# thilinarmtb/lsbench

Measured on AMD Instinct MI355X. Metric: cg_solves_per_sec, higher is better.
Workload: dtype f64

## Files before the change

lsbench_amd/csrc/hip_kernels.hip:

```cpp
#include "hip_kcommon.h"

__device__ __forceinline__ void spmv_publish(double *__restrict__ partials, double dot,
                                             double *sred, const lsb_ar_tail &tail) {
  if (!partials)
    return;
  double d[1] = {dot};
  wg_sum<1>(d, sred);
  if (tail.counter)
    ar_tail(partials, d[0], tail);
  else if (threadIdx.x == 0)
    partials[blockIdx.x] = d[0];
}

enum { SP_PREFETCH = 1, SP_NT = 2 };

template <int FLAGS, class T>
__device__ __forceinline__ T stream_load(const T *p) {
  if (FLAGS & SP_NT)
    return __builtin_nontemporal_load(p);
  return *p;
}

#define LSB_ISSUE_BLOCK(kk)                                                    \
  do {                                                                         \
// ... 602 lines not shown
        edge = x[e];
      }
      if (!have_xd && !(dot_is_x && bc == 0)) {
        if (row + 1 < n)
          xd = *(const sell_d2v *)(xdot + row);
        else if (row < n)
          xd.x = xdot[row];
        have_xd = true;
      }
      unsigned long long mk[2][2] = {{0ull, 0ull}, {0ull, 0ull}};
#pragma unroll
      for (int side = 0; side < 2; side++)
        if (side_k[side] >= 0 && side_kd[side] == 2) {
          const unsigned long long *mp = mask + 2 * ((size_t)mb + (unsigned)side_k[side]);
          mk[side][0] = mp[0], mk[side][1] = mp[1];
        }
      TMPL_UNPARK();
      if (stopped)
        return;
      double up = lane_above(c.y), dn = lane_below(c.x);
      if (lane == 0)
        up = edge;
      if (lane == 63)
        dn = edge;
      if (!have_xd)
        xd.x = c.x, xd.y = c.y, have_xd = true;
#pragma unroll
      for (int k = 0; k < NF; k++) {
        const double v = T->cst[k];
        a0 = fma(v, lo[k].x, a0), a1 = fma(v, lo[k].y, a1);
      }
      {
        double vm0 = T->cst[NF], vm1 = vm0, vp0 = T->cst[NF + 2], vp1 = vp0;
        if (side_k[0] >= 0 || side_k[1] >= 0)
          tmpl_side_values(T, NF, vb, lane, side_k, side_kd, mk, vals, f32, vm0, vm1, vp0, vp1);
        const double vc = T->cst[NF + 1];
        a0 = fma(vm0, vm0 != 0.0 ? up : 0.0, a0), a1 = fma(vm1, vm1 != 0.0 ? c.x : 0.0, a1);
        a0 = fma(vc, c.x, a0), a1 = fma(vc, c.y, a1);
        a0 = fma(vp0, vp0 != 0.0 ? c.y : 0.0, a0), a1 = fma(vp1, vp1 != 0.0 ? dn : 0.0, a1);
      }
#pragma unroll
      for (int k = 0; k < NF; k++) {
        const double v = T->cst[NF + 3 + k];
        a0 = fma(v, hi[k].x, a0), a1 = fma(v, hi[k].y, a1);
      }
    } else {
      TMPL_UNPARK();
      if (!have_xd) {
        if (row + 1 < n)
          xd = *(const sell_d2v *)(xdot + row);
        else if (row < n)
          xd.x = xdot[row];
        have_xd = true;
      }
      if (t != 255u) {
        const int cnt = T->nslots;
        if (stopped)
          return;
        for (int u0 = 0; u0 < LSB_TMPL_SLOTS; u0 += 4) {
          sell_d2u v[4];
#pragma unroll
          for (int u = 0; u < 4; u++)
            if (u0 + u < cnt)
              v[u] = *(const sell_d2u *)(x + (grow + T->base[u0 + u]));
#pragma unroll
          for (int u = 0; u < 4; u++)
            if (u0 + u < cnt) {
              const double k = T->cst[u0 + u];
              a0 = fma(k, v[u].x, a0), a1 = fma(k, v[u].y, a1);
            }
        }
      } else {
        const unsigned q0 = sptr[s] / LSB_SELL_ROWS, len = (sptr[s + 1] - sptr[s]) / LSB_SELL_ROWS;
        if (stopped)
          return;
        for (unsigned j = 0; j < len; j++) {
          const i4v r = ((const i4v *)sbase)[q0 + j];
          if (r.z < 0) {
            const double k = vconst[q0 + j];
            const sell_d2u v = *(const sell_d2u *)(x + (grow + r.x));
            a0 = fma(k, v.x, a0), a1 = fma(k, v.y, a1);
          } else {
            double v0, v1;
            if (f32) {
              const vt2<float>::type v = *((const vt2<float>::type *)((const float *)vals + (size_t)r.z * LSB_SELL_ROWS) + lane);
              v0 = (double)v.x, v1 = (double)v.y;
            } else {
              const sell_d2v v = *((const sell_d2v *)((const double *)vals + (size_t)r.z * LSB_SELL_ROWS) + lane);
              v0 = v.x, v1 = v.y;
            }
            const bool p0 = v0 != 0.0, p1 = v1 != 0.0;
            const double t0 = x[p0 ? grow + r.x : 0], t1 = x[p1 ? grow + 1 + r.x : 0];
            a0 = fma(v0, p0 ? t0 : 0.0, a0), a1 = fma(v1, p1 ? t1 : 0.0, a1);
          }
        }
      }
    }
    if (CHEB) {
      if (row + 1 < n) {
        const sell_d2v rr = *(const sell_d2v *)(epi.r + row), dd = *(const sell_d2v *)(epi.d + row);
        const double i0 = epi.dinv ? epi.dinv[row] : epi.dc, i1 = epi.dinv ? epi.dinv[row + 1] : epi.dc;
        const double v0 = fma(epi.a, dd.x, epi.b * (i0 * (rr.x - a0)));
        const double v1 = fma(epi.a, dd.y, epi.b * (i1 * (rr.y - a1)));
        const sell_d2v dn2 = {v0, v1}, zn = {x[grow] + v0, x[grow + 1] + v1};
        *(sell_d2v *)(epi.d + row) = dn2;
        *(sell_d2v *)(epi.zout + row) = zn;
      } else if (row < n) {
        const double v0 = fma(epi.a, epi.d[row], epi.b * ((epi.dinv ? epi.dinv[row] : epi.dc) * (epi.r[row] - a0)));
        epi.d[row] = v0;
        epi.zout[row] = x[grow] + v0;
      }
    } else if (DEFER && s * LSB_SELL_ROWS + LSB_SELL_ROWS <= n) {
      const sell_d2v o = {a0, a1};
      if (DEFER_DEPTH == 1 || pslot == 0)
        ypark[tid] = o, parked[0] = s * LSB_SELL_ROWS;
      else
        ypark[(DEFER_DEPTH - 1) * WG + tid] = o, parked[DEFER_DEPTH - 1] = s * LSB_SELL_ROWS;
      if (xdot) {
        dot = fma(a0, xd.x, dot);
        dot = fma(a1, xd.y, dot);
      }
    } else if (row + 1 < n) {
      const sell_d2v o = {a0, a1};
      *(sell_d2v *)(y + row) = o;
      if (xdot) {
        dot = fma(a0, xd.x, dot);
        dot = fma(a1, xd.y, dot);
      }
    } else if (row < n) {
      y[row] = a0;
      if (xdot)
        dot = fma(a0, xd.x, dot);
    }
  }
#pragma unroll
  for (int k = 0; k < DEFER_DEPTH; k++)
    TMPL_UNPARK_SLOT(k);
#undef TMPL_UNPARK
#undef TMPL_UNPARK_SLOT
  if (stopped)
    return;
  spmv_publish(partials, dot, sred, tail);
}

template <int NF> struct col_ops {
  sell_d2u lo[NF > 1 ? NF - 1 : 1], hi[NF > 1 ? NF - 1 : 1];
  double edge;
  sell_d2v xd;
};
template <int NF> struct col_tmpl {
  int bc, bl[NF > 1 ? NF - 1 : 1], bh[NF > 1 ? NF - 1 : 1];
  double k0, kl[NF > 1 ? NF - 1 : 1], kc, kh[NF > 1 ? NF - 1 : 1], kL;
};
template <int NF, int DOT>
__device__ __forceinline__ void col_issue(col_ops<NF> &o, sell_d2u &cnext, const col_tmpl<NF> &T, const double *__restrict__ x,
                                          const double *__restrict__ xdot, long long gu, unsigned lrow, long long D,
                                          unsigned xlen, unsigned lane, bool with_next) {
  if (with_next)
    cnext = *(const sell_d2u *)(x + (gu + T.bc + D) + 2 * lane);
#pragma unroll
  for (int k = 0; k < NF - 1; k++) {
    o.lo[k] = *(const sell_d2u *)(x + (gu + T.bl[k]) + 2 * lane);
    o.hi[k] = *(const sell_d2u *)(x + (gu + T.bh[k]) + 2 * lane);
  }
  long long el = gu + T.bc - 1, er = gu + T.bc + (long long)LSB_SELL_ROWS;
  el = el < 0 ? 0 : el, er = er >= (long long)xlen ? (long long)xlen - 1 : er;
  o.edge = x[lane < 32u ? el : er];
  if (DOT == 2)
    o.xd = *(const sell_d2v *)(xdot + lrow + 2 * lane);
}
template <int NF, int DOT>
__device__ __forceinline__ void col_compute(const col_ops<NF> &o, const sell_d2u &cm, const sell_d2u &c, const sell_d2u &cp,
                                            const col_tmpl<NF> &T, double vm0, double vm1, double vp0, double vp1,
                                            unsigned lane, double &a0, double &a1, double &dot) {
  double up = lane_above(c.y), dn = lane_below(c.x);
  if (lane == 0)
    up = o.edge;
  if (lane == 63)
    dn = o.edge;
  a0 = fma(T.k0, cm.x, 0.0), a1 = fma(T.k0, cm.y, 0.0);
#pragma unroll
  for (int k = 0; k < NF - 1; k++)
    a0 = fma(T.kl[k], o.lo[k].x, a0), a1 = fma(T.kl[k], o.lo[k].y, a1);
  a0 = fma(vm0, vm0 != 0.0 ? up : 0.0, a0), a1 = fma(vm1, vm1 != 0.0 ? c.x : 0.0, a1);
  a0 = fma(T.kc, c.x, a0), a1 = fma(T.kc, c.y, a1);
  a0 = fma(vp0, vp0 != 0.0 ? c.y : 0.0, a0), a1 = fma(vp1, vp1 != 0.0 ? dn : 0.0, a1);
#pragma unroll
  for (int k = 0; k < NF - 1; k++)
    a0 = fma(T.kh[k], o.hi[k].x, a0), a1 = fma(T.kh[k], o.hi[k].y, a1);
  a0 = fma(T.kL, cp.x, a0), a1 = fma(T.kL, cp.y, a1);
  if (DOT == 1)
    dot = fma(a0, c.x, dot), dot = fma(a1, c.y, dot);
  else if (DOT == 2)
    dot = fma(a0, o.xd.x, dot), dot = fma(a1, o.xd.y, dot);
}

#define LSB_COL_HEAD 16
__device__ __forceinline__ bool col_walks_down(const unsigned *__restrict__ plan, unsigned dofs, unsigned it) {
  return dofs && ((plan[dofs + (it >> 5)] >> (it & 31u)) & 1u);
}
template <int NF, int DOT>
__global__ __launch_bounds__(WG, DOT == 2 ? 5 : 6) void k_spmv_tmpl_col(
    const unsigned *__restrict__ plan, unsigned period, unsigned n, unsigned row_begin, unsigned xlen,
    const unsigned *__restrict__ sptr, const unsigned long long *__restrict__ mask,
    const lsb_sell_tmpl *__restrict__ td, const int *__restrict__ sbase, const void *__restrict__ vals, int f32,
    const double *__restrict__ vconst, const double *__restrict__ x, double *__restrict__ y,
    const double *__restrict__ xdot, double *__restrict__ partials, const lsb_pcg_state *__restrict__ st,
    const lsb_ar_tail tail) {
  static_assert(NF >= 1 && NF <= 2, "one or two far slots per side");
  __shared__ double sred[4];
  const unsigned tid = threadIdx.x, lane = tid & 63u, wave = tid >> 6;
  const unsigned gx = gridDim.x / NXCD, xcd = blockIdx.x % NXCD, slot = blockIdx.x / NXCD;
  const unsigned i0 = plan[xcd], i1 = plan[xcd + 1];
  const u4v *__restrict__ items = (const u4v *)(plan + LSB_COL_HEAD);
  const unsigned dofs = plan[LSB_TMPL_COL_DOWN];
  const int stopped = st ? st->status : 0;
  const unsigned P = period * LSB_SELL_ROWS;
  double dot = 0.0;
  for (unsigned g = slot; i0 + 4 * g < i1; g += gx) {
    const unsigned it = __builtin_amdgcn_readfirstlane(i0 + 4 * g + wave);
    if (it >= i1)
      continue;
    const u4v rec = items[it];
    const unsigned s = __builtin_amdgcn_readfirstlane(rec.x), Kw = __builtin_amdgcn_readfirstlane(rec.y);
    const unsigned K = Kw & ~LSB_TMPL_COL_LOCKSTEP;
    const bool lockstep = (Kw & LSB_TMPL_COL_LOCKSTEP) != 0;
    if (K >= 2) {
      const unsigned t = __builtin_amdgcn_readfirstlane(rec.z), mb = __builtin_amdgcn_readfirstlane(rec.w);
      const lsb_sell_tmpl *T = td + t;
      col_tmpl<NF> C;
      C.bc = T->base[NF + 1];
      C.k0 = T->cst[0], C.kc = T->cst[NF + 1], C.kL = T->cst[2 * NF + 2];
#pragma unroll
      for (int k = 0; k < NF - 1; k++) {
        C.bl[k] = T->base[1 + k], C.bh[k] = T->base[NF + 3 + k];
        C.kl[k] = T->cst[1 + k], C.kh[k] = T->cst[NF + 3 + k];
      }
      const int side_k[2] = {T->kidx[NF], T->kidx[NF + 2]}, side_kd[2] = {T->kind[NF], T->kind[NF + 2]};
      unsigned long long mk[2][2] = {{0ull, 0ull}, {0ull, 0ull}};
#pragma unroll
      for (int side = 0; side < 2; side++)
        if (side_k[side] >= 0 && side_kd[side] == 2) {
          const unsigned long long *mp = mask + 2 * ((size_t)mb + (unsigned)side_k[side]);
          mk[side][0] = mp[0], mk[side][1] = mp[1];
        }
      const bool down = col_walks_down(plan, dofs, it);
      const unsigned s0 = down ? s + (K - 1) * period : s;
      const long long D = down ? -(long long)P : (long long)P;
      const unsigned Du = (unsigned)D;
      long long gu = (long long)s0 * LSB_SELL_ROWS + row_begin;
      unsigned lrow = s0 * LSB_SELL_ROWS;
      col_ops<NF> cur, nxt;
      sell_d2u cb = *(const sell_d2u *)(x + (gu + C.bc - D) + 2 * lane);
      sell_d2u c0 = *(const sell_d2u *)(x + (gu + C.bc) + 2 * lane);
      sell_d2u ca, cn;
      col_issue<NF, DOT>(cur, ca, C, x, xdot, gu, lrow, D, xlen, lane, true);
      double vm0 = T->cst[NF], vm1 = vm0, vp0 = T->cst[NF + 2], vp1 = vp0;
      if (side_k[0] >= 0 || side_k[1] >= 0)
        tmpl_side_values(T, NF, 0u, lane, side_k, side_kd, mk, vals, f32, vm0, vm1, vp0, vp1);
      if (stopped)
        return;
      col_issue<NF, DOT>(nxt, cn, C, x, xdot, gu + D, lrow + Du, D, xlen, lane, true);
      double a0, a1;
      col_compute<NF, DOT>(cur, down ? ca : cb, c0, down ? cb : ca, C, vm0, vm1, vp0, vp1, lane, a0, a1, dot);
      cb = c0, c0 = ca, ca = cn, cur = nxt;
      for (unsigned k = 1; k + 1 < K; k++) {
        gu += D, lrow += Du;
        if (lockstep)
          __builtin_amdgcn_s_barrier();
        col_issue<NF, DOT>(nxt, cn, C, x, xdot, gu + D, lrow + Du, D, xlen, lane, true);
        {
          const sell_d2v o = {a0, a1};
          *(sell_d2v *)(y + (lrow - Du) + 2 * lane) = o;
        }
        col_compute<NF, DOT>(cur, down ? ca : cb, c0, down ? cb : ca, C, vm0, vm1, vp0, vp1, lane, a0, a1, dot);
        cb = c0, c0 = ca, ca = cn, cur = nxt;
      }
      gu += D, lrow += Du;
      {
        const sell_d2v o = {a0, a1};
        *(sell_d2v *)(y + (lrow - Du) + 2 * lane) = o;
      }
      col_compute<NF, DOT>(cur, down ? ca : cb, c0, down ? cb : ca, C, vm0, vm1, vp0, vp1, lane, a0, a1, dot);
      {
        const sell_d2v o = {a0, a1};
        *(sell_d2v *)(y + lrow + 2 * lane) = o;
      }
      if (stopped)
        return;
    } else {
      const unsigned row = s * LSB_SELL_ROWS + 2 * lane;
      const int grow = (int)(row + row_begin);
      const unsigned q0 = sptr[s] / LSB_SELL_ROWS, len = (sptr[s + 1] - sptr[s]) / LSB_SELL_ROWS;
      sell_d2v xd = {0.0, 0.0};
      if (DOT) {
        if (row + 1 < n)
          xd = *(const sell_d2v *)(xdot + row);
        else if (row < n)
          xd.x = xdot[row];
      }
      if (stopped)
        return;
      double a0 = 0.0, a1 = 0.0;
      for (unsigned j = 0; j < len; j++) {
        const i4v r = ((const i4v *)sbase)[q0 + j];
        if (r.z < 0) {
          const double k = vconst[q0 + j];
          const sell_d2u v = *(const sell_d2u *)(x + (grow + r.x));
          a0 = fma(k, v.x, a0), a1 = fma(k, v.y, a1);
        } else {
          double v0, v1;
          if (f32) {
            const vt2<float>::type v = *((const vt2<float>::type *)((const float *)vals + (size_t)r.z * LSB_SELL_ROWS) + lane);
            v0 = (double)v.x, v1 = (double)v.y;
          } else {
            const sell_d2v v = *((const sell_d2v *)((const double *)vals + (size_t)r.z * LSB_SELL_ROWS) + lane);
            v0 = v.x, v1 = v.y;
          }
          const bool p0 = v0 != 0.0, p1 = v1 != 0.0;
          const double t0 = x[p0 ? grow + r.x : 0], t1 = x[p1 ? grow + 1 + r.x : 0];
          a0 = fma(v0, p0 ? t0 : 0.0, a0), a1 = fma(v1, p1 ? t1 : 0.0, a1);
        }
      }
      if (row + 1 < n) {
        const sell_d2v o = {a0, a1};
        *(sell_d2v *)(y + row) = o;
        if (DOT)
          dot = fma(a0, xd.x, dot), dot = fma(a1, xd.y, dot);
      } else if (row < n) {
        y[row] = a0;
        if (DOT)
          dot = fma(a0, xd.x, dot);
      }
    }
  }
  if (stopped)
    return;
  spmv_publish(partials, dot, sred, tail);
}

template <int NF> struct colp_c {
  sell_d2u rn, pn;
  sell_d2v xn, sn;
  double re, pe;
};
template <int NF> struct colp_m {
  sell_d2u rlo[NF > 1 ? NF - 1 : 1], plo[NF > 1 ? NF - 1 : 1], rhi[NF > 1 ? NF - 1 : 1], phi[NF > 1 ? NF - 1 : 1];
};
struct colp_out {
  sell_d2v q, x, p;
};
template <int NF, bool WITH_X, int NT>
__device__ __forceinline__ void colp_issue_c(colp_c<NF> &o, const col_tmpl<NF> &T, const double *__restrict__ r,
                                             const double *__restrict__ pold, const double *__restrict__ x,
                                             const double *pstale, long long gu, long long D, unsigned xlen,
                                             unsigned lane) {
  const long long ga = gu + T.bc + D;
  o.rn = *(const sell_d2u *)(r + ga + 2 * lane);
  o.pn = *(const sell_d2u *)(pold + ga + 2 * lane);
  if (WITH_X) {
    if (NT & 1) {
      o.xn = __builtin_nontemporal_load((const sell_d2v *)(x + (gu + D) + 2 * lane));
      o.sn = __builtin_nontemporal_load((const sell_d2v *)(pstale + (gu + D) + 2 * lane));
    } else {
      o.xn = *(const sell_d2v *)(x + (gu + D) + 2 * lane);
      o.sn = *(const sell_d2v *)(pstale + (gu + D) + 2 * lane);
    }
  }
  long long el = gu + T.bc - 1, er = gu + T.bc + (long long)LSB_SELL_ROWS;
  el = el < 0 ? 0 : el, er = er >= (long long)xlen ? (long long)xlen - 1 : er;
  const long long e = lane < 32u ? el : er;
  o.re = r[e], o.pe = pold[e];
}
template <int NF>
__device__ __forceinline__ void colp_issue_m(colp_m<NF> &o, const col_tmpl<NF> &T, const double *__restrict__ r,
                                             const double *__restrict__ pold, long long gu, unsigned lane) {
#pragma unroll
  for (int k = 0; k < NF - 1; k++) {
    o.rlo[k] = *(const sell_d2u *)(r + (gu + T.bl[k]) + 2 * lane);
    o.plo[k] = *(const sell_d2u *)(pold + (gu + T.bl[k]) + 2 * lane);
    o.rhi[k] = *(const sell_d2u *)(r + (gu + T.bh[k]) + 2 * lane);
    o.phi[k] = *(const sell_d2u *)(pold + (gu + T.bh[k]) + 2 * lane);
  }
}
template <int NF, bool OWNED, bool XUPD>
__device__ __forceinline__ void colp_compute(const colp_c<NF> &o, const colp_m<NF> &m, const sell_d2u &pb,
                                             const sell_d2u &p0, sell_d2u &pp, bool down, const col_tmpl<NF> &T, double vm0,
                                             double vm1, double vp0, double vp1, double beta, double alpha, double alpha2,
                                             double dc, unsigned lane, colp_out &out, double &dot) {
  pp.x = pnew_of(dc, o.rn.x, beta, o.pn.x), pp.y = pnew_of(dc, o.rn.y, beta, o.pn.y);
  if (OWNED) {
    if (XUPD) {
      out.x.x = (o.xn.x + alpha2 * o.sn.x) + alpha * o.pn.x, out.x.y = (o.xn.y + alpha2 * o.sn.y) + alpha * o.pn.y;
    }
    out.p.x = pp.x, out.p.y = pp.y;
  }
  const double edge = pnew_of(dc, o.re, beta, o.pe);
  double up = lane_above(p0.y), dn = lane_below(p0.x);
  if (lane == 0)
    up = edge;
  if (lane == 63)
    dn = edge;
  const sell_d2u &pm = down ? pp : pb, &pu = down ? pb : pp;
  double a0 = fma(T.k0, pm.x, 0.0), a1 = fma(T.k0, pm.y, 0.0);
#pragma unroll
  for (int k = 0; k < NF - 1; k++) {
    const double l0 = pnew_of(dc, m.rlo[k].x, beta, m.plo[k].x), l1 = pnew_of(dc, m.rlo[k].y, beta, m.plo[k].y);
    a0 = fma(T.kl[k], l0, a0), a1 = fma(T.kl[k], l1, a1);
  }
  a0 = fma(vm0, vm0 != 0.0 ? up : 0.0, a0), a1 = fma(vm1, vm1 != 0.0 ? p0.x : 0.0, a1);
  a0 = fma(T.kc, p0.x, a0), a1 = fma(T.kc, p0.y, a1);
  a0 = fma(vp0, vp0 != 0.0 ? p0.y : 0.0, a0), a1 = fma(vp1, vp1 != 0.0 ? dn : 0.0, a1);
#pragma unroll
  for (int k = 0; k < NF - 1; k++) {
    const double h0 = pnew_of(dc, m.rhi[k].x, beta, m.phi[k].x), h1 = pnew_of(dc, m.rhi[k].y, beta, m.phi[k].y);
    a0 = fma(T.kh[k], h0, a0), a1 = fma(T.kh[k], h1, a1);
  }
  a0 = fma(T.kL, pu.x, a0), a1 = fma(T.kL, pu.y, a1);
  out.q.x = a0, out.q.y = a1;
  dot = fma(a0, p0.x, dot), dot = fma(a1, p0.y, dot);
}
__device__ __forceinline__ void colp_single(unsigned s, unsigned n, unsigned lane, const unsigned *__restrict__ sptr,
                                            const int *__restrict__ sbase, const double *__restrict__ vals,
                                            const double *__restrict__ vconst, const double *__restrict__ r,
                                            const double *__restrict__ pold, double *pnew,
                                            double *__restrict__ x, double *__restrict__ q, double beta, double alpha,
                                            double alpha2, bool xupd, double dc, double &dot) {
  const unsigned row = s * LSB_SELL_ROWS + 2 * lane;
  const unsigned q0 = sptr[s] / LSB_SELL_ROWS, len = (sptr[s + 1] - sptr[s]) / LSB_SELL_ROWS;
  const bool l0 = row < n, l1 = row + 1 < n;
  const double r0 = l0 ? r[row] : 0.0, r1 = l1 ? r[row + 1] : 0.0;
  const double o0 = l0 ? pold[row] : 0.0, o1 = l1 ? pold[row + 1] : 0.0;
  const double x0 = xupd && l0 ? x[row] : 0.0, x1 = xupd && l1 ? x[row + 1] : 0.0;
  const double s0 = xupd && l0 ? pnew[row] : 0.0, s1 = xupd && l1 ? pnew[row + 1] : 0.0;
  double a0 = 0.0, a1 = 0.0;
  for (unsigned j = 0; j < len; j++) {
    const i4v rec = ((const i4v *)sbase)[q0 + j];
    if (rec.z < 0) {
      const double k = vconst[q0 + j];
      const sell_d2u rv = *(const sell_d2u *)(r + ((int)row + rec.x)), pv = *(const sell_d2u *)(pold + ((int)row + rec.x));
      a0 = fma(k, pnew_of(dc, rv.x, beta, pv.x), a0), a1 = fma(k, pnew_of(dc, rv.y, beta, pv.y), a1);
    } else {
      const sell_d2v v = *((const sell_d2v *)(vals + (size_t)rec.z * LSB_SELL_ROWS) + lane);
      const bool p0 = v.x != 0.0, p1 = v.y != 0.0;
      const int c0 = p0 ? (int)row + rec.x : 0, c1 = p1 ? (int)row + 1 + rec.x : 0;
      const double t0 = pnew_of(dc, r[c0], beta, pold[c0]), t1 = pnew_of(dc, r[c1], beta, pold[c1]);
      a0 = fma(v.x, p0 ? t0 : 0.0, a0), a1 = fma(v.y, p1 ? t1 : 0.0, a1);
    }
  }
  const double n0 = pnew_of(dc, r0, beta, o0), n1 = pnew_of(dc, r1, beta, o1);
  if (l0) {
    pnew[row] = n0;
    if (xupd)
      x[row] = (x0 + alpha2 * s0) + alpha * o0;
    if (q)
      q[row] = a0;
    dot = fma(a0, n0, dot);
  }
  if (l1) {
    pnew[row + 1] = n1;
    if (xupd)
      x[row + 1] = (x1 + alpha2 * s1) + alpha * o1;
    if (q)
      q[row + 1] = a1;
    dot = fma(a1, n1, dot);
  }
}

#define COLP_ST(PTR, V, BIT)                                                                   \
  do {                                                                                         \
    if (NT & (BIT))                                                                            \
      __builtin_nontemporal_store((V), (sell_d2v *)(PTR));                                     \
    else                                                                                       \
      *(sell_d2v *)(PTR) = (V);                                                                \
  } while (0)
#define COLP_STORE(OUT, LROW, WITH_Q, WITH_XP)                                                 \
  do {                                                                                         \
    if (WITH_Q)                                                                                \
      COLP_ST(q + (LROW) + 2 * lane, (OUT).q, 2);                                              \
    if (WITH_XP) {                                                                             \
      if (XUPD)                                                                                \
        COLP_ST(x + ((LROW) + Du) + 2 * lane, (OUT).x, 1);                                     \
      COLP_ST(pnew + ((LROW) + Du) + 2 * lane, (OUT).p, 2);                                    \
    }                                                                                          \
  } while (0)

template <int NF, int NT, bool XUPD>
__global__ __launch_bounds__(WG, NF == 2 ? 3 : 5) void k_pcg_col_px(
    const unsigned *__restrict__ plan, unsigned period, unsigned n, const unsigned *__restrict__ sptr,
    const unsigned long long *__restrict__ mask, const lsb_sell_tmpl *__restrict__ td, const int *__restrict__ sbase,
    const double *__restrict__ vals, const double *__restrict__ vconst, const double *__restrict__ r,
    const double *__restrict__ pold, double *pnew, double *__restrict__ x, double dc,
    double *__restrict__ partials, lsb_pcg_state *__restrict__ st, int parity,
    const double *__restrict__ parts2, unsigned nparts2) {
  static_assert(NF >= 1 && NF <= 2, "one or two far slots per side");
  __shared__ double sred[8];
  double *const q = nullptr;
  const unsigned tid = threadIdx.x, lane = tid & 63u, wave = tid >> 6;
  const unsigned gx = gridDim.x / NXCD, xcd = blockIdx.x % NXCD, slot = blockIdx.x / NXCD;
  const int stopped = st->status;
  const double rz_old = st->rz[parity], thresh2 = st->thresh2, alpha = st->alpha[0], alpha2 = st->alpha[1];
  const unsigned i0 = plan[xcd], i1 = plan[xcd + 1];
  double v[2];
  wg_sum_partials<2>(parts2, nparts2, v, sred);
  if (stopped)
    return;
  const double rz_new = v[0], rr = v[1];
  const bool conv = rr <= thresh2;
  if (blockIdx.x == 0 && threadIdx.x == 0) {
    const int it = st->iters + 1;
    st->iters = it;
    st->rr = rr;
    st->rz[parity ^ 1] = rz_new;
    if (conv)
      st->status = LSB_STATUS_CONVERGED;
    else {
      if (XUPD)
        st->xpend = 0;
      if (it >= st->maxit)
        st->pad = 1;
    }
  }
  if (conv)
    return;
  const double beta = rz_new / rz_old;
  const u4v *__restrict__ items = (const u4v *)(plan + LSB_COL_HEAD);
  const unsigned dofs = plan[LSB_TMPL_COL_DOWN];
  const unsigned P = period * LSB_SELL_ROWS;
  double dot = 0.0;
  for (unsigned g = slot; i0 + 4 * g < i1; g += gx) {
    const unsigned it = __builtin_amdgcn_readfirstlane(i0 + 4 * g + wave);
    if (it >= i1)
      continue;
    const u4v rec = items[it];
    const unsigned s = __builtin_amdgcn_readfirstlane(rec.x);
    const unsigned K = __builtin_amdgcn_readfirstlane(rec.y) & ~LSB_TMPL_COL_LOCKSTEP;
    if (K >= 3) {
      const unsigned t = __builtin_amdgcn_readfirstlane(rec.z), mb = __builtin_amdgcn_readfirstlane(rec.w);
      const lsb_sell_tmpl *T = td + t;
      col_tmpl<NF> C;
      C.bc = T->base[NF + 1];
      C.k0 = T->cst[0], C.kc = T->cst[NF + 1], C.kL = T->cst[2 * NF + 2];
#pragma unroll
      for (int k = 0; k < NF - 1; k++) {
        C.bl[k] = T->base[1 + k], C.bh[k] = T->base[NF + 3 + k];
        C.kl[k] = T->cst[1 + k], C.kh[k] = T->cst[NF + 3 + k];
      }
      const int side_k[2] = {T->kidx[NF], T->kidx[NF + 2]}, side_kd[2] = {T->kind[NF], T->kind[NF + 2]};
      const bool down = col_walks_down(plan, dofs, it);
      const unsigned s0 = down ? s + (K - 1) * period : s;
      const long long D = down ? -(long long)P : (long long)P;
      const unsigned Du = (unsigned)D;
      long long gu = (long long)s0 * LSB_SELL_ROWS;
      unsigned lrow = s0 * LSB_SELL_ROWS;
      const long long gc = gu + C.bc;
      const sell_d2u rb = *(const sell_d2u *)(r + (gc - D) + 2 * lane);
      const sell_d2u pb = *(const sell_d2u *)(pold + (gc - D) + 2 * lane);
      const sell_d2u r0 = *(const sell_d2u *)(r + gc + 2 * lane), o0 = *(const sell_d2u *)(pold + gc + 2 * lane);
      sell_d2v x0 = {0.0, 0.0}, s0v = {0.0, 0.0};
      if (XUPD)
        x0 = *(const sell_d2v *)(x + lrow + 2 * lane), s0v = *(const sell_d2v *)(pnew + lrow + 2 * lane);
      colp_c<NF> c0, c1;
      colp_m<NF> m0, m1, m2;
      colp_issue_c<NF, XUPD, NT>(c0, C, r, pold, x, pnew, gu, D, n, lane);
      colp_issue_m<NF>(m0, C, r, pold, gu, lane);
      colp_issue_m<NF>(m1, C, r, pold, gu + D, lane);
      unsigned long long mk[2][2] = {{0ull, 0ull}, {0ull, 0ull}};
#pragma unroll
      for (int side = 0; side < 2; side++)
        if (side_k[side] >= 0 && side_kd[side] == 2) {
          const unsigned long long *mp = mask + 2 * ((size_t)mb + (unsigned)side_k[side]);
          mk[side][0] = mp[0], mk[side][1] = mp[1];
        }
      double vm0 = T->cst[NF], vm1 = vm0, vp0 = T->cst[NF + 2], vp1 = vp0;
      if (side_k[0] >= 0 || side_k[1] >= 0)
        tmpl_side_values(T, NF, 0u, lane, side_k, side_kd, mk, vals, 0, vm0, vm1, vp0, vp1);
      sell_d2u pm, p0, pp;
      pm.x = pnew_of(dc, rb.x, beta, pb.x), pm.y = pnew_of(dc, rb.y, beta, pb.y);
      p0.x = pnew_of(dc, r0.x, beta, o0.x), p0.y = pnew_of(dc, r0.y, beta, o0.y);
      colp_out res;
      res.x.x = (x0.x + alpha2 * s0v.x) + alpha * o0.x, res.x.y = (x0.y + alpha2 * s0v.y) + alpha * o0.y;
      res.p.x = p0.x, res.p.y = p0.y;
      res.q = res.p;
      COLP_STORE(res, lrow - Du, false, true);
      for (unsigned k = 0; k + 2 < K; k++) {
        colp_issue_c<NF, XUPD, NT>(c1, C, r, pold, x, pnew, gu + D, D, n, lane);
        colp_issue_m<NF>(m2, C, r, pold, gu + 2 * D, lane);
        colp_compute<NF, true, XUPD>(c0, m0, pm, p0, pp, down, C, vm0, vm1, vp0, vp1, beta, alpha, alpha2, dc, lane, res, dot);
        COLP_STORE(res, lrow, false, true);
        pm = p0, p0 = pp, c0 = c1, m0 = m1, m1 = m2;
        gu += D, lrow += Du;
      }
      colp_issue_c<NF, false, NT>(c1, C, r, pold, x, pnew, gu + D, D, n, lane);
      colp_compute<NF, true, XUPD>(c0, m0, pm, p0, pp, down, C, vm0, vm1, vp0, vp1, beta, alpha, alpha2, dc, lane, res, dot);
      COLP_STORE(res, lrow, false, true);
      pm = p0, p0 = pp, c0 = c1, m0 = m1;
      gu += D, lrow += Du;
      colp_compute<NF, false, XUPD>(c0, m0, pm, p0, pp, down, C, vm0, vm1, vp0, vp1, beta, alpha, alpha2, dc, lane, res, dot);
      COLP_STORE(res, lrow, false, false);
    } else {
      for (unsigned k = 0; k < K; k++)
        colp_single(s + k * period, n, lane, sptr, sbase, vals, vconst, r, pold, pnew, x, nullptr, beta, alpha, alpha2,
                    XUPD, dc, dot);
    }
  }
  if (partials) {
    double d[1] = {dot};
    wg_sum<1>(d, sred);
    if (threadIdx.x == 0)
      partials[blockIdx.x] = d[0];
  }
}
#undef COLP_STORE
#undef COLP_ST

template <int NF>
__global__ __launch_bounds__(WG, 5) void k_pcg_col_r(
    const unsigned *__restrict__ plan, unsigned period, unsigned n, const unsigned *__restrict__ sptr,
    const unsigned long long *__restrict__ mask, const lsb_sell_tmpl *__restrict__ td, const int *__restrict__ sbase,
    const double *__restrict__ vals, const double *__restrict__ vconst, const double *__restrict__ p,
    double *__restrict__ r, double dc, lsb_pcg_state *__restrict__ st, int parity, int pbuf, int xtwo, int rev,
    const double *__restrict__ pq_parts, unsigned npq, double *__restrict__ partials2) {
  static_assert(NF >= 1 && NF <= 2, "one or two far slots per side");
  __shared__ double sred[8];
  const unsigned tid = threadIdx.x, lane = tid & 63u, wave = tid >> 6;
  const unsigned gx = gridDim.x / NXCD, xcd = blockIdx.x % NXCD, slot = blockIdx.x / NXCD;
  const int stopped = st->status, pad = st->pad;
  const double rz = st->rz[parity];
  const unsigned i0 = plan[xcd], i1 = plan[xcd + 1];
  double pqv[1];
  wg_sum_partials<1>(pq_parts, npq, pqv, sred);
  if (stopped)
    return;
  if (pad) {
    if (blockIdx.x == 0 && threadIdx.x == 0)
      st->status = LSB_STATUS_MAXIT;
    return;
  }
  const double pq = pqv[0];
  if (!(pq != 0.0) || !isfinite(pq)) {
    if (blockIdx.x == 0 && threadIdx.x == 0)
      st->status = LSB_STATUS_BREAKDOWN;
    return;
  }
  const double alpha = rz / pq;
  if (blockIdx.x == 0 && threadIdx.x == 0) {
    st->pq = pq, st->alpha[1] = st->alpha[0], st->alpha[0] = alpha, st->xpend = (xtwo ? 3 : 1) + pbuf;
  }
  const u4v *__restrict__ items = (const u4v *)(plan + LSB_COL_HEAD);
  const unsigned dofs = plan[LSB_TMPL_COL_DOWN];
  const unsigned P = period * LSB_SELL_ROWS;
  double acc[2] = {0.0, 0.0}, nodot = 0.0;
#define COLR_FINISH(A0, A1, RV, LROW)                                                          \
  do {                                                                                         \
    sell_d2v rn_;                                                                              \
    rn_.x = (RV).x - alpha * (A0), rn_.y = (RV).y - alpha * (A1);                              \
    *(sell_d2v *)(r + (LROW) + 2 * lane) = rn_;                                                \
    acc[0] += rn_.x * (dc * rn_.x);                                                            \
    acc[0] += rn_.y * (dc * rn_.y);                                                            \
    acc[1] += rn_.x * rn_.x;                                                                   \
    acc[1] += rn_.y * rn_.y;                                                                   \
  } while (0)
  const unsigned G = (i1 - i0 + 3u) / 4u;
  for (unsigned j = slot; j < G; j += gx) {
    const unsigned g = rev ? G - 1u - j : j;
    const unsigned it = __builtin_amdgcn_readfirstlane(i0 + 4 * g + wave);
    if (it >= i1)
      continue;
    const u4v rec = items[it];
    const unsigned s = __builtin_amdgcn_readfirstlane(rec.x);
    const unsigned K = __builtin_amdgcn_readfirstlane(rec.y) & ~LSB_TMPL_COL_LOCKSTEP;
    if (K >= 3) {
      const unsigned t = __builtin_amdgcn_readfirstlane(rec.z), mb = __builtin_amdgcn_readfirstlane(rec.w);
      const lsb_sell_tmpl *T = td + t;
      col_tmpl<NF> C;
      C.bc = T->base[NF + 1];
      C.k0 = T->cst[0], C.kc = T->cst[NF + 1], C.kL = T->cst[2 * NF + 2];
#pragma unroll
      for (int k = 0; k < NF - 1; k++) {
        C.bl[k] = T->base[1 + k], C.bh[k] = T->base[NF + 3 + k];
        C.kl[k] = T->cst[1 + k], C.kh[k] = T->cst[NF + 3 + k];
      }
      const int side_k[2] = {T->kidx[NF], T->kidx[NF + 2]}, side_kd[2] = {T->kind[NF], T->kind[NF + 2]};
      const bool down = col_walks_down(plan, dofs, it);
      const unsigned s0 = down ? s + (K - 1) * period : s;
      const long long D = down ? -(long long)P : (long long)P;
      const unsigned Du = (unsigned)D;
      long long gu = (long long)s0 * LSB_SELL_ROWS;
      unsigned lrow = s0 * LSB_SELL_ROWS;
      col_ops<NF> cur, nxt;
      sell_d2u cb = *(const sell_d2u *)(p + (gu + C.bc - D) + 2 * lane);
      sell_d2u c0 = *(const sell_d2u *)(p + (gu + C.bc) + 2 * lane);
      sell_d2u ca, cn;
      col_issue<NF, 2>(cur, ca, C, p, r, gu, lrow, D, n, lane, true);
      unsigned long long mk[2][2] = {{0ull, 0ull}, {0ull, 0ull}};
#pragma unroll
      for (int side = 0; side < 2; side++)
        if (side_k[side] >= 0 && side_kd[side] == 2) {
          const unsigned long long *mp = mask + 2 * ((size_t)mb + (unsigned)side_k[side]);
          mk[side][0] = mp[0], mk[side][1] = mp[1];
        }
      double vm0 = T->cst[NF], vm1 = vm0, vp0 = T->cst[NF + 2], vp1 = vp0;
      if (side_k[0] >= 0 || side_k[1] >= 0)
        tmpl_side_values(T, NF, 0u, lane, side_k, side_kd, mk, vals, 0, vm0, vm1, vp0, vp1);
      for (unsigned k = 0; k + 1 < K; k++) {
        col_issue<NF, 2>(nxt, cn, C, p, r, gu + D, lrow + Du, D, n, lane, true);
        double a0, a1;
        col_compute<NF, 0>(cur, down ? ca : cb, c0, down ? cb : ca, C, vm0, vm1, vp0, vp1, lane, a0, a1, nodot);
        COLR_FINISH(a0, a1, cur.xd, lrow);
        cb = c0, c0 = ca, ca = cn, cur = nxt;
        gu += D, lrow += Du;
      }
      double a0, a1;
      col_compute<NF, 0>(cur, down ? ca : cb, c0, down ? cb : ca, C, vm0, vm1, vp0, vp1, lane, a0, a1, nodot);
      COLR_FINISH(a0, a1, cur.xd, lrow);
    } else {
      for (unsigned k = 0; k < K; k++) {
        const unsigned sl = s + k * period, row = sl * LSB_SELL_ROWS + 2 * lane;
        const unsigned q0 = sptr[sl] / LSB_SELL_ROWS, len = (sptr[sl + 1] - sptr[sl]) / LSB_SELL_ROWS;
        const bool l0 = row < n, l1 = row + 1 < n;
        const double r0 = l0 ? r[row] : 0.0, r1 = l1 ? r[row + 1] : 0.0;
        double a0 = 0.0, a1 = 0.0;
        for (unsigned j = 0; j < len; j++) {
          const i4v rec2 = ((const i4v *)sbase)[q0 + j];
          if (rec2.z < 0) {
            const double kk = vconst[q0 + j];
            const sell_d2u pv = *(const sell_d2u *)(p + ((int)row + rec2.x));
            a0 = fma(kk, pv.x, a0), a1 = fma(kk, pv.y, a1);
          } else {
            const sell_d2v v = *((const sell_d2v *)(vals + (size_t)rec2.z * LSB_SELL_ROWS) + lane);
            const bool p0 = v.x != 0.0, p1 = v.y != 0.0;
            const double t0 = p[p0 ? (int)row + rec2.x : 0], t1 = p[p1 ? (int)row + 1 + rec2.x : 0];
            a0 = fma(v.x, p0 ? t0 : 0.0, a0), a1 = fma(v.y, p1 ? t1 : 0.0, a1);
          }
        }
        if (l0) {
          const double rn0 = r0 - alpha * a0;
          r[row] = rn0;
          acc[0] += rn0 * (dc * rn0), acc[1] += rn0 * rn0;
        }
        if (l1) {
          const double rn1 = r1 - alpha * a1;
          r[row + 1] = rn1;
          acc[0] += rn1 * (dc * rn1), acc[1] += rn1 * rn1;
        }
      }
    }
  }
#undef COLR_FINISH
  wg_sum<2>(acc, sred);
  if (threadIdx.x == 0) {
    partials2[2 * blockIdx.x + 0] = acc[0];
    partials2[2 * blockIdx.x + 1] = acc[1];
  }
}


__device__ __forceinline__ unsigned bin_pad(unsigned i) { return i + (i >> 3); }

template <int FLAGS, int BIN_U>
__global__ __launch_bounds__(WG) void k_spmv_binned(
    const unsigned *__restrict__ chunk_begin, unsigned nchunk, const unsigned *__restrict__ rows,
    const unsigned *__restrict__ cols, const double *__restrict__ vals,
    const double *__restrict__ x, double *__restrict__ y, const lsb_pcg_state *__restrict__ st) {
  constexpr unsigned CHUNK = BIN_U * WG;
  __shared__ double sprod[CHUNK + CHUNK / 8 + 8];
  __shared__ unsigned skey[CHUNK + CHUNK / 8 + 8];
  __shared__ double swv[4];
  __shared__ int swf[4];
  __shared__ double sred[4];
  const unsigned tid = threadIdx.x, lane = tid & 63u, wave = tid >> 6;
  const unsigned per = gridDim.x / NXCD;
  const unsigned w = (blockIdx.x % NXCD) * per + blockIdx.x / NXCD;
  if (w >= nchunk)
    return;
  const unsigned e0 = chunk_begin[w], cnt = chunk_begin[w + 1] - e0;
  unsigned r[BIN_U], c[BIN_U];
  double v[BIN_U];
  if (cnt <= CHUNK) {
#pragma unroll
    for (int u = 0; u < BIN_U; u++) {
      const unsigned t = tid + u * WG;
      if (t < cnt) {
        r[u] = stream_load<FLAGS>(rows + e0 + t);
        c[u] = stream_load<FLAGS>(cols + e0 + t);
        v[u] = stream_load<FLAGS>(vals + e0 + t);
      }
    }
  }
  if (st && st->status)
    return;
  if (cnt > CHUNK) {
    double s[1] = {0.0};
    for (unsigned j = e0 + tid; j < e0 + cnt; j += WG)
      s[0] += vals[j] * x[cols[j]];
    wg_sum<1>(s, sred);
    if (tid == 0)
      y[rows[e0]] += s[0];
    return;
  }
#pragma unroll
  for (int u = 0; u < BIN_U; u++) {
    const unsigned t = tid + u * WG;
    if (t < cnt) {
      double xv;
      if (FLAGS & 8)
        xv = __hip_atomic_load(x + c[u], __ATOMIC_RELAXED, __HIP_MEMORY_SCOPE_AGENT);
      else if (FLAGS & 16)
        xv = __builtin_nontemporal_load(x + c[u]);
      else
        xv = x[c[u]];
      sprod[bin_pad(t)] = v[u] * xv;
      skey[bin_pad(t)] = r[u];
    }
  }
  __syncthreads();
  const unsigned i0 = tid * BIN_U;
  const int nloc = i0 < cnt ? (int)min(cnt - i0, (unsigned)BIN_U) : 0;
  double first_sum = 0.0, acc = 0.0;
  unsigned first_key = 0, prevk = 0xFFFFFFFFu, nextk = 0xFFFFFFFEu;
  bool cont = false, has_boundary = false, closes = true;
  unsigned ok_[BIN_U];
  double ov[BIN_U];
  unsigned omask = 0;
  if (nloc > 0) {
    if (i0 > 0)
      prevk = skey[bin_pad(i0 - 1)];
    if (i0 + BIN_U < cnt)
      nextk = skey[bin_pad(i0 + BIN_U)];
    unsigned k[BIN_U + 1];
    double p[BIN_U];
#pragma unroll
    for (int j = 0; j < BIN_U; j++) {
      k[j] = j < nloc ? skey[bin_pad(i0 + j)] : 0u;
      p[j] = j < nloc ? sprod[bin_pad(i0 + j)] : 0.0;
    }
    cont = k[0] == prevk;
    first_key = k[0];
#pragma unroll
    for (int j = 0; j < BIN_U; j++)
      if (j < nloc) {
        acc += p[j];
        const bool last = j == nloc - 1;
        const bool ends = last ? (k[j] != nextk) : (k[j + 1] != k[j]);
        if (last)
          closes = ends;
        if (ends) {
          if (cont && !has_boundary) {
            first_sum = acc;
          } else {
            omask |= 1u << j;
            ok_[j] = k[j], ov[j] = acc;
          }
          if (!last)
            has_boundary = true, acc = 0.0;
        }
      }
    double yv[BIN_U];
#pragma unroll
// ... 297 lines not shown
```

Measured before the change: 1.121.

## Prefetch partials and first column header before grid reduction in fused PCG kernels

In the fused PCG column kernels, the loads of the reduction partials are issued into registers before the state reads, and for NF==1 the first work item's template header is loaded before the workgroup reduction, so their latency overlaps the reduction. The r-update kernel also switches to nontemporal loads and stores for the residual vector. This targets the serialized latency at kernel start after the cross-block reduction. In exchange it raises register pressure, which may reduce occupancy, and the nontemporal hints may hurt if r would otherwise be reused from cache.

Result: slower. 0.9367 (-16.4%).

```diff
diff --git a/lsbench_amd/csrc/hip_kernels.hip b/lsbench_amd/csrc/hip_kernels.hip
--- a/lsbench_amd/csrc/hip_kernels.hip
+++ b/lsbench_amd/csrc/hip_kernels.hip
@@ -778,7 +778,7 @@
   int bc, bl[NF > 1 ? NF - 1 : 1], bh[NF > 1 ? NF - 1 : 1];
   double k0, kl[NF > 1 ? NF - 1 : 1], kc, kh[NF > 1 ? NF - 1 : 1], kL;
 };
-template <int NF, int DOT>
+template <int NF, int DOT, bool NTD = false>
 __device__ __forceinline__ void col_issue(col_ops<NF> &o, sell_d2u &cnext, const col_tmpl<NF> &T, const double *__restrict__ x,
                                           const double *__restrict__ xdot, long long gu, unsigned lrow, long long D,
                                           unsigned xlen, unsigned lane, bool with_next) {
@@ -792,8 +792,12 @@
   long long el = gu + T.bc - 1, er = gu + T.bc + (long long)LSB_SELL_ROWS;
   el = el < 0 ? 0 : el, er = er >= (long long)xlen ? (long long)xlen - 1 : er;
   o.edge = x[lane < 32u ? el : er];
-  if (DOT == 2)
-    o.xd = *(const sell_d2v *)(xdot + lrow + 2 * lane);
+  if (DOT == 2) {
+    if (NTD)
+      o.xd = __builtin_nontemporal_load((const sell_d2v *)(xdot + lrow + 2 * lane));
+    else
+      o.xd = *(const sell_d2v *)(xdot + lrow + 2 * lane);
+  }
 }
 template <int NF, int DOT>
 __device__ __forceinline__ void col_compute(const col_ops<NF> &o, const sell_d2u &cm, const sell_d2u &c, const sell_d2u &cp,
@@ -824,6 +828,101 @@
 #define LSB_COL_HEAD 16
 __device__ __forceinline__ bool col_walks_down(const unsigned *__restrict__ plan, unsigned dofs, unsigned it) {
   return dofs && ((plan[dofs + (it >> 5)] >> (it & 31u)) & 1u);
+}
+template <int NF> struct col_head {
+  unsigned s, K, mb;
+  col_tmpl<NF> C;
+  int side_k[2], side_kd[2];
+  double vm, vp;
+};
+template <int NF>
+__device__ __forceinline__ void col_head_load(col_head<NF> &h, const u4v *__restrict__ items,
+                                              const lsb_sell_tmpl *__restrict__ td, unsigned it) {
+  const u4v rec = items[it];
+  h.s = __builtin_amdgcn_readfirstlane(rec.x);
+  h.K = __builtin_amdgcn_readfirstlane(rec.y) & ~LSB_TMPL_COL_LOCKSTEP;
+  const unsigned t = h.K >= 3 ? __builtin_amdgcn_readfirstlane(rec.z) : 0u;
+  h.mb = __builtin_amdgcn_readfirstlane(rec.w);
+  const lsb_sell_tmpl *T = td + t;
+  h.C.bc = T->base[NF + 1];
+  h.C.k0 = T->cst[0], h.C.kc = T->cst[NF + 1], h.C.kL = T->cst[2 * NF + 2];
+#pragma unroll
+  for (int k = 0; k < NF - 1; k++) {
+    h.C.bl[k] = T->base[1 + k], h.C.bh[k] = T->base[NF + 3 + k];
+    h.C.kl[k] = T->cst[1 + k], h.C.kh[k] = T->cst[NF + 3 + k];
+  }
+  h.side_k[0] = T->kidx[NF], h.side_k[1] = T->kidx[NF + 2];
+  h.side_kd[0] = T->kind[NF], h.side_kd[1] = T->kind[NF + 2];
+  h.vm = T->cst[NF], h.vp = T->cst[NF + 2];
+}
+template <int NF>
+__device__ __forceinline__ void col_head_side_values(const col_head<NF> &h, unsigned lane,
+                                                     const unsigned long long *__restrict__ mask,
+                                                     const double *__restrict__ vals, double &vm0, double &vm1,
+                                                     double &vp0, double &vp1) {
+  unsigned long long mk[2][2] = {{0ull, 0ull}, {0ull, 0ull}};
+#pragma unroll
+  for (int side = 0; side < 2; side++)
+    if (h.side_k[side] >= 0 && h.side_kd[side] == 2) {
+      const unsigned long long *mp = mask + 2 * ((size_t)h.mb + (unsigned)h.side_k[side]);
+      mk[side][0] = mp[0], mk[side][1] = mp[1];
+    }
+  vm0 = vm1 = h.vm, vp0 = vp1 = h.vp;
+#pragma unroll
+  for (int side = 0; side < 2; side++) {
+    const int k = h.side_k[side];
+    if (k < 0)
+      continue;
+    const double c = side == 0 ? h.vm : h.vp;
+    double v0, v1;
+    if (h.side_kd[side] == 2) {
+      const unsigned long long w = (lane & 32u) ? mk[side][1] : mk[side][0];
+      const unsigned sh = (2u * lane) & 63u;
+      v0 = (w >> sh) & 1ull ? c : 0.0;
+      v1 = (w >> (sh + 1u)) & 1ull ? c : 0.0;
+    } else {
+      const sell_d2v v = *((const sell_d2v *)(vals + (size_t)(unsigned)k * LSB_SELL_ROWS) + lane);
+      v0 = v.x, v1 = v.y;
+    }
+    if (side == 0)
+      vm0 = v0, vm1 = v1;
+    else
+      vp0 = v0, vp1 = v1;
+  }
+}
+#define COL_PARTS_U 5
+template <int W> struct col_parts {
+  double v[COL_PARTS_U][W];
+};
+template <int W>
+__device__ __forceinline__ void col_parts_issue(col_parts<W> &ph, const double *__restrict__ parts, unsigned nparts) {
+#pragma unroll
+  for (int u = 0; u < COL_PARTS_U; u++) {
+    const unsigned i = threadIdx.x + u * WG, ic = i < nparts ? i : 0u;
+#pragma unroll
+    for (int k = 0; k < W; k++)
+      ph.v[u][k] = parts[(size_t)ic * W + k];
+  }
+}
+template <int W>
+__device__ __forceinline__ void col_parts_sum(const col_parts<W> &ph, const double *__restrict__ parts, unsigned nparts,
+                                              double (&v)[W], double *sred) {
+#pragma unroll
+  for (int k = 0; k < W; k++)
+    v[k] = 0.0;
+#pragma unroll
+  for (int u = 0; u < COL_PARTS_U; u++)
+    if (threadIdx.x + u * WG < nparts) {
+#pragma unroll
+      for (int k = 0; k < W; k++)
+        v[k] += ph.v[u][k];
+    }
+  for (unsigned i = threadIdx.x + COL_PARTS_U * WG; i < nparts; i += WG) {
+#pragma unroll
+    for (int k = 0; k < W; k++)
+      v[k] += parts[(size_t)i * W + k];
+  }
+  wg_sum<W>(v, sred);
 }
 template <int NF, int DOT>
 __global__ __launch_bounds__(WG, DOT == 2 ? 5 : 6) void k_spmv_tmpl_col(
@@ -1124,11 +1223,22 @@
   double *const q = nullptr;
   const unsigned tid = threadIdx.x, lane = tid & 63u, wave = tid >> 6;
   const unsigned gx = gridDim.x / NXCD, xcd = blockIdx.x % NXCD, slot = blockIdx.x / NXCD;
+  col_parts<2> ph;
+  col_parts_issue<2>(ph, parts2, nparts2);
   const int stopped = st->status;
   const double rz_old = st->rz[parity], thresh2 = st->thresh2, alpha = st->alpha[0], alpha2 = st->alpha[1];
   const unsigned i0 = plan[xcd], i1 = plan[xcd + 1];
+  const u4v *__restrict__ items = (const u4v *)(plan + LSB_COL_HEAD);
+  const unsigned dofs = plan[LSB_TMPL_COL_DOWN];
+  constexpr bool EARLY = NF == 1;
+  col_head<NF> h = {};
+  {
+    const unsigned it = __builtin_amdgcn_readfirstlane(i0 + 4 * slot + wave);
+    if (EARLY && i0 + 4 * slot < i1 && it < i1)
+      col_head_load<NF>(h, items, td, it);
+  }
   double v[2];
-  wg_sum_partials<2>(parts2, nparts2, v, sred);
+  col_parts_sum<2>(ph, parts2, nparts2, v, sred);
   if (stopped)
     return;
   const double rz_new = v[0], rr = v[1];
@@ -1150,29 +1260,17 @@
   if (conv)
     return;
   const double beta = rz_new / rz_old;
-  const u4v *__restrict__ items = (const u4v *)(plan + LSB_COL_HEAD);
-  const unsigned dofs = plan[LSB_TMPL_COL_DOWN];
   const unsigned P = period * LSB_SELL_ROWS;
   double dot = 0.0;
   for (unsigned g = slot; i0 + 4 * g < i1; g += gx) {
     const unsigned it = __builtin_amdgcn_readfirstlane(i0 + 4 * g + wave);
     if (it >= i1)
       continue;
-    const u4v rec = items[it];
-    const unsigned s = __builtin_amdgcn_readfirstlane(rec.x);
-    const unsigned K = __builtin_amdgcn_readfirstlane(rec.y) & ~LSB_TMPL_COL_LOCKSTEP;
+    if (!EARLY || g != slot)
+      col_head_load<NF>(h, items, td, it);
+    const unsigned s = h.s, K = h.K;
     if (K >= 3) {
-      const unsigned t = __builtin_amdgcn_readfirstlane(rec.z), mb = __builtin_amdgcn_readfirstlane(rec.w);
-      const lsb_sell_tmpl *T = td + t;
-      col_tmpl<NF> C;
-      C.bc = T->base[NF + 1];
-      C.k0 = T->cst[0], C.kc = T->cst[NF + 1], C.kL = T->cst[2 * NF + 2];
-#pragma unroll
-      for (int k = 0; k < NF - 1; k++) {
-        C.bl[k] = T->base[1 + k], C.bh[k] = T->base[NF + 3 + k];
-        C.kl[k] = T->cst[1 + k], C.kh[k] = T->cst[NF + 3 + k];
-      }
-      const int side_k[2] = {T->kidx[NF], T->kidx[NF + 2]}, side_kd[2] = {T->kind[NF], T->kind[NF + 2]};
+      const col_tmpl<NF> &C = h.C;
       const bool down = col_walks_down(plan, dofs, it);
       const unsigned s0 = down ? s + (K - 1) * period : s;
       const long long D = down ? -(long long)P : (long long)P;
@@ -1191,16 +1289,8 @@
       colp_issue_c<NF, XUPD, NT>(c0, C, r, pold, x, pnew, gu, D, n, lane);
       colp_issue_m<NF>(m0, C, r, pold, gu, lane);
       colp_issue_m<NF>(m1, C, r, pold, gu + D, lane);
-      unsigned long long mk[2][2] = {{0ull, 0ull}, {0ull, 0ull}};
-#pragma unroll
-      for (int side = 0; side < 2; side++)
-        if (side_k[side] >= 0 && side_kd[side] == 2) {
-          const unsigned long long *mp = mask + 2 * ((size_t)mb + (unsigned)side_k[side]);
-          mk[side][0] = mp[0], mk[side][1] = mp[1];
-        }
-      double vm0 = T->cst[NF], vm1 = vm0, vp0 = T->cst[NF + 2], vp1 = vp0;
-      if (side_k[0] >= 0 || side_k[1] >= 0)
-        tmpl_side_values(T, NF, 0u, lane, side_k, side_kd, mk, vals, 0, vm0, vm1, vp0, vp1);
+      double vm0, vm1, vp0, vp1;
+      col_head_side_values<NF>(h, lane, mask, vals, vm0, vm1, vp0, vp1);
       sell_d2u pm, p0, pp;
       pm.x = pnew_of(dc, rb.x, beta, pb.x), pm.y = pnew_of(dc, rb.y, beta, pb.y);
       p0.x = pnew_of(dc, r0.x, beta, o0.x), p0.y = pnew_of(dc, r0.y, beta, o0.y);
@@ -1251,11 +1341,23 @@
   __shared__ double sred[8];
   const unsigned tid = threadIdx.x, lane = tid & 63u, wave = tid >> 6;
   const unsigned gx = gridDim.x / NXCD, xcd = blockIdx.x % NXCD, slot = blockIdx.x / NXCD;
+  col_parts<1> ph;
+  col_parts_issue<1>(ph, pq_parts, npq);
   const int stopped = st->status, pad = st->pad;
   const double rz = st->rz[parity];
   const unsigned i0 = plan[xcd], i1 = plan[xcd + 1];
+  const u4v *__restrict__ items = (const u4v *)(plan + LSB_COL_HEAD);
+  const unsigned dofs = plan[LSB_TMPL_COL_DOWN];
+  const unsigned G = (i1 - i0 + 3u) / 4u;
+  constexpr bool EARLY = NF == 1;
+  col_head<NF> h = {};
+  {
+    const unsigned it = __builtin_amdgcn_readfirstlane(i0 + 4 * (rev ? G - 1u - slot : slot) + wave);
+    if (EARLY && slot < G && it < i1)
+      col_head_load<NF>(h, items, td, it);
+  }
   double pqv[1];
-  wg_sum_partials<1>(pq_parts, npq, pqv, sred);
+  col_parts_sum<1>(ph, pq_parts, npq, pqv, sred);
   if (stopped)
     return;
   if (pad) {
@@ -1273,41 +1375,28 @@
   if (blockIdx.x == 0 && threadIdx.x == 0) {
     st->pq = pq, st->alpha[1] = st->alpha[0], st->alpha[0] = alpha, st->xpend = (xtwo ? 3 : 1) + pbuf;
   }
-  const u4v *__restrict__ items = (const u4v *)(plan + LSB_COL_HEAD);
-  const unsigned dofs = plan[LSB_TMPL_COL_DOWN];
   const unsigned P = period * LSB_SELL_ROWS;
   double acc[2] = {0.0, 0.0}, nodot = 0.0;
 #define COLR_FINISH(A0, A1, RV, LROW)                                                          \
   do {                                                                                         \
     sell_d2v rn_;                                                                              \
     rn_.x = (RV).x - alpha * (A0), rn_.y = (RV).y - alpha * (A1);                              \
-    *(sell_d2v *)(r + (LROW) + 2 * lane) = rn_;                                                \
+    __builtin_nontemporal_store(rn_, (sell_d2v *)(r + (LROW) + 2 * lane));                     \
     acc[0] += rn_.x * (dc * rn_.x);                                                            \
     acc[0] += rn_.y * (dc * rn_.y);                                                            \
     acc[1] += rn_.x * rn_.x;                                                                   \
     acc[1] += rn_.y * rn_.y;                                                                   \
   } while (0)
-  const unsigned G = (i1 - i0 + 3u) / 4u;
   for (unsigned j = slot; j < G; j += gx) {
     const unsigned g = rev ? G - 1u - j : j;
     const unsigned it = __builtin_amdgcn_readfirstlane(i0 + 4 * g + wave);
     if (it >= i1)
       continue;
-    const u4v rec = items[it];
-    const unsigned s = __builtin_amdgcn_readfirstlane(rec.x);
-    const unsigned K = __builtin_amdgcn_readfirstlane(rec.y) & ~LSB_TMPL_COL_LOCKSTEP;
+    if (!EARLY || j != slot)
+      col_head_load<NF>(h, items, td, it);
+    const unsigned s = h.s, K = h.K;
     if (K >= 3) {
-      const unsigned t = __builtin_amdgcn_readfirstlane(rec.z), mb = __builtin_amdgcn_readfirstlane(rec.w);
-      const lsb_sell_tmpl *T = td + t;
-      col_tmpl<NF> C;
-      C.bc = T->base[NF + 1];
-      C.k0 = T->cst[0], C.kc = T->cst[NF + 1], C.kL = T->cst[2 * NF + 2];
-#pragma unroll
-      for (int k = 0; k < NF - 1; k++) {
-        C.bl[k] = T->base[1 + k], C.bh[k] = T->base[NF + 3 + k];
-        C.kl[k] = T->cst[1 + k], C.kh[k] = T->cst[NF + 3 + k];
-      }
-      const int side_k[2] = {T->kidx[NF], T->kidx[NF + 2]}, side_kd[2] = {T->kind[NF], T->kind[NF + 2]};
+      const col_tmpl<NF> &C = h.C;
       const bool down = col_walks_down(plan, dofs, it);
       const unsigned s0 = down ? s + (K - 1) * period : s;
       const long long D = down ? -(long long)P : (long long)P;
@@ -1318,19 +1407,11 @@
       sell_d2u cb = *(const sell_d2u *)(p + (gu + C.bc - D) + 2 * lane);
       sell_d2u c0 = *(const sell_d2u *)(p + (gu + C.bc) + 2 * lane);
       sell_d2u ca, cn;
-      col_issue<NF, 2>(cur, ca, C, p, r, gu, lrow, D, n, lane, true);
-      unsigned long long mk[2][2] = {{0ull, 0ull}, {0ull, 0ull}};
-#pragma unroll
-      for (int side = 0; side < 2; side++)
-        if (side_k[side] >= 0 && side_kd[side] == 2) {
-          const unsigned long long *mp = mask + 2 * ((size_t)mb + (unsigned)side_k[side]);
-          mk[side][0] = mp[0], mk[side][1] = mp[1];
-        }
-      double vm0 = T->cst[NF], vm1 = vm0, vp0 = T->cst[NF + 2], vp1 = vp0;
-      if (side_k[0] >= 0 || side_k[1] >= 0)
-        tmpl_side_values(T, NF, 0u, lane, side_k, side_kd, mk, vals, 0, vm0, vm1, vp0, vp1);
+      col_issue<NF, 2, true>(cur, ca, C, p, r, gu, lrow, D, n, lane, true);
+      double vm0, vm1, vp0, vp1;
+      col_head_side_values<NF>(h, lane, mask, vals, vm0, vm1, vp0, vp1);
       for (unsigned k = 0; k + 1 < K; k++) {
-        col_issue<NF, 2>(nxt, cn, C, p, r, gu + D, lrow + Du, D, n, lane, true);
+        col_issue<NF, 2, true>(nxt, cn, C, p, r, gu + D, lrow + Du, D, n, lane, true);
         double a0, a1;
         col_compute<NF, 0>(cur, down ? ca : cb, c0, down ? cb : ca, C, vm0, vm1, vp0, vp1, lane, a0, a1, nodot);
         COLR_FINISH(a0, a1, cur.xd, lrow);
```
